# theadamsabra/last_torch

Hardware: AMD Instinct MI355X
Metric: lattice cells/s (B·T·U·|ctx|) at T=1000,U=100; 1/2/4/8-GPU scaling (higher is better)
Workload: dtype f32; 1 GPU; Log-semiring forward-backward (loss + dW), B=64/GPU, T=1000, U=100, V=32, FullNGram n=1 (C=33), fp32 (BASELINE configs[1]; configs[2] at 8 GPUs); batch_per_gpu=64, global_batch=64, frames=1000, labels=100, vocab=32, context_size=1, context_states=33, parallelism=utterance-sharded x1 (LPT), one RCCL all-reduce per step

## Files before the change

### last_torch_amd/csrc/lt_chunk.hip

```cpp
#include "lt_kernels.h"

#include <unistd.h>

#include <atomic>
#include <chrono>

namespace {

typedef float v16f __attribute__((ext_vector_type(16)));

constexpr float kEmin = 0x1p-88f;
constexpr int kRec = 1248;
constexpr int kRowT = 36;
constexpr int kChunkLds = 40 * 1024;
constexpr int kMargWaves = 4;
constexpr int kGrp = 7;
constexpr float kCert = 64.f;
constexpr int kAbWaves = 3;
constexpr unsigned kSpinMax = 1u << 20;
constexpr int kWalkPrio = 3;
constexpr int kDenPrio = 3;
constexpr int kASlot = 5 * 1024;
constexpr int kALdsBytes = 4 * 2 * kASlot;
constexpr int kWalkSlots = 3;
constexpr int kRecNi = (4 * kRec + 1023) / 1024;
constexpr int kWalkSlot = kRecNi * 1024;
constexpr int kWalkLds = 2 * kWalkSlots * kWalkSlot;
constexpr int kRecEj = 1152, kRecRt = 1184, kRecRho = 1216, kRecPi = 1217, kRecCs = 1218,
              kRecFlag = 1219, kRecN = 1220;

struct CkArgs {
  const unsigned char* W;
  const int* nfr;
  const int* labels;
  const int* nlab;
  const float* grad;
  float* rec;
  float* nb;
  int* uflag;
  float* abd;
  float* bbd;
  float* nabd;
  float* nbbd;
  float* cf;
  unsigned long long* ready;
  unsigned long long* prog;
  unsigned long long ep_tag, pg_tag;
  float* mid;
  float* loss;
  float* log_z;
  float* num;
  float* lz_out;
  float* num_out;
  void* dW;
  int B, T, U, V, C, R, FR, NP, NPG, PPL, CP;
  int L, K;
  int NGc;
  int nc, wpos;
  int nbs;
  int half;
  int cont;
  int local;
  int strict;
  int dbg;
  long long* stamps;
  long long FB;
  int a_slots, a_ni, a_slot_bytes, a_wave_bytes, a_off_rt, a_off_tab;
  int b_ni, b_slots, b_off_ra, b_off_rb, b_off_ga, b_off_gb, b_gslots, b_gslot, b_off_buf;
  int c_ni, c_off_ad, c_off_bd, c_off_an, c_off_bn, c_off_nw, c_off_fs, c_off_tab, c_off_cf,
      c_off_buf, c_off_fl, c_off_e, c_bytes;
};

LT_DEVINL float half_sum(float v) {
  auto p = __builtin_amdgcn_permlane32_swap(__float_as_int(v), __float_as_int(v), false, false);
  return __int_as_float(p[0]) + __int_as_float(p[1]);
}
LT_DEVINL float half_max(float v) {
  auto p = __builtin_amdgcn_permlane32_swap(__float_as_int(v), __float_as_int(v), false, false);
  float r;
  asm("v_max_f32 %0, %1, %2" : "=v"(r) : "v"(__int_as_float(p[0])), "v"(__int_as_float(p[1])));
  return r;
}
LT_DEVINL float from_prev(float v, float fill) {
  return __int_as_float(
      __builtin_amdgcn_update_dpp(__float_as_int(fill), __float_as_int(v), 0x138, 0xF, 0xF, false));
}
LT_DEVINL float rot_prev(float v) {
  return __int_as_float(__builtin_amdgcn_update_dpp(0, __float_as_int(v), 0x13C, 0xF, 0xF, false));
}
LT_DEVINL float rot_next(float v) {
  return __int_as_float(__builtin_amdgcn_update_dpp(0, __float_as_int(v), 0x134, 0xF, 0xF, false));
}

LT_DEVINL float safe_max(float m) { return __builtin_isfinite(m) ? m : 0.f; }
#ifdef LT_DIAG
#define CK_STAMP(k)                                                                  \
  do {                                                                               \
    if (a.stamps && !LT_ABL(a, 64 | 256) && threadIdx.x == 0)                         \
      a.stamps[(long long)blockIdx.x * 8 + (k)] = (long long)__builtin_amdgcn_s_memtime(); \
  } while (0)
#define CK_WSTAMP(k)                                                                 \
  do {                                                                               \
    if (a.stamps && LT_ABL(a, 64) && (threadIdx.x & 63) == 0)                         \
      a.stamps[(long long)b * 8 + (k)] = (long long)__builtin_amdgcn_s_memtime();     \
  } while (0)
#define CK_ASTAMP(k)                                                                 \
  do {                                                                               \
    if (a.stamps && LT_ABL(a, 256) && (threadIdx.x & 63) == 0)                        \
      a.stamps[(long long)a.B * a.K * 8 + (long long)id * 4 + (k)] =                  \
          (long long)__builtin_amdgcn_s_memtime();                                   \
  } while (0)
#else
#define CK_ASTAMP(k) \
  do {               \
  } while (0)
#define CK_WSTAMP(k) \
  do {               \
  } while (0)
#define CK_STAMP(k) \
  do {              \
  } while (0)
#endif
LT_DEVINL float max3_raw(float x, float y, float z) {
  float r;
  asm("v_max3_f32 %0, %1, %2, %3" : "=v"(r) : "v"(x), "v"(y), "v"(z));
  return r;
}
LT_DEVINL float first_lane(float v) {
  return __int_as_float(__builtin_amdgcn_readfirstlane(__float_as_int(v)));
}

LT_DEVINL int kstep(int s, int h) { return (s & 3) + 8 * (s >> 2) + 4 * h; }

template <bool BF16>
LT_DEVINL float ldsw(const unsigned char* fr, int e) {
  if constexpr (BF16) return __uint_as_float(((unsigned)((const unsigned short*)fr)[e]) << 16);
  else return ((const float*)fr)[e];
}

LT_DEVINL void dma_issue(const unsigned char* base, long long off, long long bytes,
                         unsigned lds_addr, int ni, int lane, int wave0 = 0, int nwaves = 1,
                         bool sc1 = false) {
  const long long a0 = off & ~15LL;
  const int n16 = (int)((off + bytes - a0 + 15) >> 4);
  for (int i = wave0; i < ni; i += nwaves) {
    int g = lane + 64 * i;
    g = g < n16 ? g : n16 - 1;
    if (sc1) glds16_sc1(base + a0 + 16LL * g, lds_addr + 1024u * i);
    else glds16(base + a0 + 16LL * g, lds_addr + 1024u * i);
  }
}

template <bool MAX>
LT_DEVINL float wred(float v) {
  if constexpr (MAX) v = dpp_max<3>(dpp_max<2>(dpp_max<1>(dpp_max<0>(v))));
  else v = dpp_add<3>(dpp_add<2>(dpp_add<1>(dpp_add<0>(v))));
  return __int_as_float(__builtin_amdgcn_readlane(__float_as_int(rows_fold<MAX>(v)), 63));
}
LT_DEVINL float wmax_u(float v) { return wred<true>(v); }
LT_DEVINL float wsum_u(float v) { return wred<false>(v); }

template <bool BF16>
LT_DEVINL float ldg(const unsigned char* base, long long e) {
  if constexpr (BF16) return __uint_as_float(((unsigned)((const unsigned short*)base)[e]) << 16);
  else return ((const float*)base)[e];
}

LT_DEVINL void string_offsets(const CkArgs& a, const int* lab, int u, int* boff, int* loff) {
  auto valid = [&](int y) { return y >= 1 && y <= a.V; };
  int ctx = 0, pc = 0;
  int j = min(u, a.U) - 1;
  for (; j >= 0; --j)
    if (valid(lab[j])) { ctx = lab[j]; break; }
  if (u >= 1) {
    if (j == u - 1) {
      for (int i = u - 2; i >= 0; --i)
        if (valid(lab[i])) { pc = lab[i]; break; }
    } else {
      pc = ctx;
    }
  }
  *boff = u < a.NP ? ctx * a.R : -1;
  if (u == 0 || u >= a.NP) {
    *loff = -1;
  } else {
    const int y = lab[u - 1];
    *loff = pc * a.R + (valid(y) ? y : 1);
  }
}

LT_DEVINL float lse2_b2(float x, float y) {
  const float m = fmaxf(x, y), n = fminf(x, y);
// ... 202 lines not shown
    const float dgv = (FULL || i < V) ? (noexp ? F.wdg : lt_exp_off(F.wdg, cl)) : 0.f;
    if (lane < 32) sdg[lane] = dgv;
    float A[16];
    float e0;
    if (noexp) {
#pragma unroll
      for (int s = 0; s < 16; ++s) A[s] = F.w[s];
      e0 = F.wr0;
    } else {
    const float ebl = lt_exp_off(F.wbl, cl);
    bool lnan = (lane <= V) && !(ebl >= 0.f);
    bool lwide = (lane <= V) && !(ebl >= kEmin);
#pragma unroll
    for (int s = 0; s < 16; ++s) {
      const bool live = FULL || (kstep(s, h) < V && i < V);
      const float e = lt_exp_off(F.w[s], cl);
      lnan = lnan || (live && !(e >= 0.f));
      lwide = lwide || (live && !(e >= kEmin));
      A[s] = live ? e : 0.f;
    }
    const float e0r = lt_exp_off(F.wr0, cl);
    e0 = (FULL || i < V) ? e0r : 0.f;
    lnan = lnan || ((FULL || i < V) && !(e0r >= 0.f));
    lwide = lwide || ((FULL || i < V) && !(e0r >= kEmin));
    if (!cfin || __builtin_amdgcn_ballot_w64(lnan)) bad = 2;
    else if (bad == 0 && __builtin_amdgcn_ballot_w64(lwide)) bad = 3;
    }
    const float w00 = F.w00;
    if (reload && !LT_ABL(a, 8192)) {
      wait_vmcnt(f + 2 < nt ? a.a_ni : 0);
      lds_frame<BF16, PPL, FULL>(aframe(f + 1), fo, F);
    }

    {
      float part = h ? 0.f : dgv * rt[i];
#pragma unroll
      for (int g = 0; g < 4; ++g) {
        const float4 r4 = *(const float4*)(rt + 8 * g + 4 * h);
        part = __builtin_fmaf(A[4 * g + 0], r4.x, part);
        part = __builtin_fmaf(A[4 * g + 1], r4.y, part);
        part = __builtin_fmaf(A[4 * g + 2], r4.z, part);
        part = __builtin_fmaf(A[4 * g + 3], r4.w, part);
      }
      const float y = half_sum(part);
      const float lam = pi;
      const int B0 = __builtin_isfinite(lam) ? max(rho, (int)floorf(lam)) : rho;
      float nr = ldexpf(y, max(rho - B0, -200)) + e0 * __builtin_amdgcn_exp2f(lam - (float)B0);
      nr = (FULL || i < V) ? nr : 0.f;
      int e;
      frexpf(wmax_u(lane < 32 ? nr : 0.f), &e);
      nr = ldexpf(nr, -e);
      rho = B0 + e;
      if (lane < 32) rt[lane] = nr;
    }
    pi += __builtin_fmaf(w00, kLog2e, -cl);
    csum += cl;

    if (LT_ABL(a, 2048)) return;
    v16f D = {};
#pragma unroll
    for (int s = 0; s < 16; ++s) D = __builtin_amdgcn_mfma_f32_32x32x2f32(A[s], X[s], D, 0, 0, 0);
#pragma unroll
    for (int g = 0; g < 4; ++g) {
      const float4 d4 = *(const float4*)(sdg + 8 * g + 4 * h);
      D[4 * g + 0] = __builtin_fmaf(d4.x, X[4 * g + 0], D[4 * g + 0]);
      D[4 * g + 1] = __builtin_fmaf(d4.y, X[4 * g + 1], D[4 * g + 1]);
      D[4 * g + 2] = __builtin_fmaf(d4.z, X[4 * g + 2], D[4 * g + 2]);
      D[4 * g + 3] = __builtin_fmaf(d4.w, X[4 * g + 3], D[4 * g + 3]);
    }
    float cm = fmaxf(max3_raw(D[0], D[1], D[2]), max3_raw(D[3], D[4], D[5]));
#pragma unroll
    for (int r = 6; r < 16; r += 2) cm = max3_raw(cm, D[r], D[r + 1]);
    cm = half_max(cm);
    int e;
    frexpf(cm, &e);
    e = cm > 0.f ? e : 0;
#pragma unroll
    for (int r = 0; r < 16; ++r) X[r] = ldexpf(D[r], -e);
    ej += e;
  };
  aissue(0);
  if (nt > 1) aissue(1);
  wait_vmcnt(nt > 1 ? a.a_ni : 0);
  lds_frame<BF16, PPL, FULL>(aframe(0), fo, fr);
  for (int f = 0; f < nt; ++f) step(fr, f, f + 1 < nt);
  if (lane < nt) a.cf[(long long)b * a.T + t0 + lane] = cfl_lane;
  CK_ASTAMP(2);

  const __amdgpu_buffer_rsrc_t rr = wt_rsrc(a.rec + (long long)id * kRec, 4 * kRec);
#pragma unroll
  for (int r = 0; r < 16; ++r) {
    st_wt(rr, kstep(r, h) * kRowT + i, X[r]);
  }
  if (lane < 32) {
    st_wt(rr, kRecEj + lane, ej);
    st_wt(rr, kRecRt + lane, rt[lane]);
  }
  bad = __builtin_amdgcn_readfirstlane(bad);
  if (lane == 0) {
    st_wt(rr, kRecRho, rho);
    st_wt(rr, kRecPi, pi);
    st_wt(rr, kRecCs, csum);
    st_wt(rr, kRecFlag, bad);
    st_wt(rr, kRecN, nt);
  }
  asm volatile("s_waitcnt vmcnt(0)" ::: "memory");
  CK_ASTAMP(3);
  const bool withhold = LT_ABL(a, 512) && b == 0 && k == 1;
  if (lane == 0 && !withhold)
    __hip_atomic_store((gu64*)(a.ready + id), a.ep_tag | (bad ? (unsigned)bad : 1u),
                       __ATOMIC_RELAXED, __HIP_MEMORY_SCOPE_AGENT);
}

LT_DEVINL unsigned long long poll_flag(const unsigned long long* p) {
  unsigned long long v;
  asm volatile("global_load_dwordx2 %0, %1, off sc1\n\ts_waitcnt vmcnt(0)" : "=v"(v) : "v"(p) : "memory");
  return v;
}
LT_DEVINL unsigned flag_state(unsigned long long v, unsigned long long tag) {
  return (v & ~3ull) == tag ? (unsigned)(v & 3) : 0u;
}
LT_DEVINL int prog_count(unsigned long long v, unsigned long long tag) {
  return (v & ~0xFFFFFFull) == tag ? (int)(v & 0xFFFFFF) : 0;
}
LT_DEVINL float4 ld_sc1x4(__amdgpu_buffer_rsrc_t r, int byte_off) {
  const v4u v = __builtin_amdgcn_raw_buffer_load_b128(r, byte_off, 0, 0x10);
  return make_float4(__uint_as_float(v.x), __uint_as_float(v.y), __uint_as_float(v.z),
                     __uint_as_float(v.w));
}
LT_DEVINL float ld_sc1(const float* p) {
  return __hip_atomic_load(p, __ATOMIC_RELAXED, __HIP_MEMORY_SCOPE_AGENT);
}
struct ChunkReady {
  const unsigned long long* f;
  unsigned long long tag;
  int lo, hi, Kl, ok, bad, strict;
  LT_DEVINL ChunkReady(const unsigned long long* flags, unsigned long long tg, int kl, int st)
      : f(flags), tag(tg), lo(kl), hi(-1), Kl(kl), ok(1), bad(0), strict(st) {}
  LT_DEVINL void take(unsigned v, int lane, int* c) {
    const unsigned long long m = __builtin_amdgcn_ballot_w64(v != 0);
    *c = m == ~0ull ? 64 : __builtin_ctzll(~m);
    const unsigned long long live = *c == 64 ? ~0ull : ((1ull << *c) - 1);
    if (__builtin_amdgcn_ballot_w64(v == 2u || (strict && v == 3u)) & live) bad = 1;
  }
  LT_DEVINL void timeout() {
    ok = 0;
    hi = Kl - 1;
    lo = 0;
  }
  LT_DEVINL void ensure_fwd(int k, int lane) {
    k = min(k, Kl - 1);
    for (unsigned spins = 0; k > hi; ++spins) {
      const int x = hi + 1 + lane;
      const unsigned v = flag_state(poll_flag(f + min(x, Kl - 1)), tag) & (x < Kl ? ~0u : 0u);
      int c;
      take(v, lane, &c);
      if (c) {
        hi += c;
      } else if (spins > kSpinMax) {
        timeout();
      } else {
        __builtin_amdgcn_s_sleep(4);
      }
    }
  }
  LT_DEVINL void ensure_bwd(int k, int lane) {
    k = max(k, 0);
    for (unsigned spins = 0; k < lo; ++spins) {
      const int x = lo - 1 - lane;
      const unsigned v = flag_state(poll_flag(f + max(x, 0)), tag) & (x >= 0 ? ~0u : 0u);
      int c;
      take(v, lane, &c);
      if (c) {
        lo -= c;
      } else if (spins > kSpinMax) {
        timeout();
      } else {
        __builtin_amdgcn_s_sleep(4);
      }
    }
  }
};

struct RecAlpha {
  float4 x[8];
  float rt, sc;
  float pi, cs;
};
LT_DEVINL void load_rec_alpha(const float* rc, int lane, int V, RecAlpha& r) {
#pragma unroll
  for (int g = 0; g < 8; ++g) r.x[g] = *(const float4*)(rc + (lane & 31) * kRowT + 4 * g);
  r.rt = rc[kRecRt + (lane & 31)];
  const int si = lane == 0 ? kRecRho : kRecEj + min(lane, 32) - 1;
  const int sc = ((const int*)rc)[si];
  r.sc = lane <= V ? (float)sc : 0.f;
  r.pi = rc[kRecPi];
  r.cs = rc[kRecCs];
}
struct RecBeta {
  float x[16];
// ... 123 lines not shown
      n[r][0] = g[r][0].x; n[r][1] = g[r][0].y; n[r][2] = g[r][0].z; n[r][3] = g[r][0].w;
      n[r][4] = g[r][1].x; n[r][5] = g[r][1].y; n[r][6] = g[r][1].z; n[r][7] = g[r][1].w;
    }
    if constexpr (FWD) {
#pragma unroll
      for (int r = 0; r < PPL; ++r)
#pragma unroll
        for (int d = 0; d < NB; ++d) tab[(lane + 64 * r + d) * TS + d] = v[r] + n[r][d];
    } else {
#pragma unroll
      for (int r = 0; r < PPL; ++r) sv[lane + 64 * r] = v[r];
    }
    __builtin_amdgcn_s_waitcnt(0xc07f);
    __builtin_amdgcn_wave_barrier();
    float x[PPL][NB];
#pragma unroll
    for (int r = 0; r < PPL; ++r)
#pragma unroll
      for (int d = 0; d < NB; ++d)
        x[r][d] = FWD ? tab[(lane + 64 * r) * TS + d] : n[r][d] + sv[lane + 64 * r + d];
    bload(qn, g);
    float vm = -kInf;
#pragma unroll
    for (int r = 0; r < PPL; ++r) {
      float m = x[r][0];
#pragma unroll
      for (int d = 1; d < NB; ++d) m = fmaxf(m, x[r][d]);
      const float ms = m == -kInf ? 0.f : m;
      float sum = 0.f;
#pragma unroll
      for (int d = 0; d < NB; ++d) sum += __builtin_amdgcn_exp2f(x[r][d] - ms);
      v[r] = lane + 64 * r < NPG ? ms + __builtin_amdgcn_logf(sum) : -kInf;
      vm = fmaxf(vm, v[r]);
    }
    {
      const float mv = wmax_u(vm);
      const float fl = __builtin_isfinite(mv) ? floorf(mv) : 0.f;
#pragma unroll
      for (int r = 0; r < PPL; ++r) v[r] -= fl;
      off += fl;
    }
    if (!FWD && q % NGc == 0) {
#pragma unroll
      for (int r = 0; r < PPL; ++r)
        if (lane + 64 * r < NPG) bd_store(dst + (long long)(q / NGc) * NPG + lane + 64 * r, v[r], wt);
      publish(Kh - q / NGc, false);
    }
    __builtin_amdgcn_wave_barrier();
  };
  const int cnt = q1 - q0;
  auto qof = [&](int n) { return FWD ? q0 + n : q1 - 1 - n; };
#pragma unroll
  for (int d = 0; d < D; ++d) bload(qof(d), gq[d]);
  const int nmain = cnt - cnt % D;
  for (int n0 = 0; n0 < nmain; n0 += D) {
#pragma unroll
    for (int d = 0; d < D; ++d) step(gq[d], qof(n0 + d), qof(n0 + d + D));
  }
#pragma unroll
  for (int d = 0; d < D; ++d)
    if (nmain + d < cnt) step(gq[d], qof(nmain + d), qof(nmain + d));
  if (ph == kWalkFirst) {
    if (FWD) {
#pragma unroll
      for (int r = 0; r < PPL; ++r)
        if (lane + 64 * r < NPG) dst[(long long)Kh * NPG + lane + 64 * r] = v[r];
      if (lane == 0) a.mid[2LL * b + 1] = off;
    }
    return;
  }
  publish(FWD ? (Kl - 1) - Kh : Kh, true);
  if constexpr (FWD) {
    float nv = -kInf;
#pragma unroll
    for (int r = 0; r < PPL; ++r)
      if (lane + 64 * r == nl) nv = v[r];
    nv = wmax_u(nv);
    if (lane == 0)
      *s_num = (nl >= 0 && nl <= a.U) ? (float)(((double)off + (double)nv) * 0.6931471805599453)
                                       : -kInf;
  }
}

template <int PPL, int D>
LT_DEVINL void combine_role(const CkArgs& a, int b, int wave, unsigned char* dyn, int ph) {
  const WalkLds wl = walk_lds(dyn);
  const int lane = threadIdx.x & 63;
  int nf = a.nfr[b];
  nf = nf < 0 ? 0 : (nf > a.T ? a.T : nf);
  const int Kl = (nf + a.L - 1) / a.L;
  const int Kh = Kl / 2;
  const int V = a.V, C = a.C, CP = a.CP;
  const int nl = a.nlab[b];
  if (ph == kWalkRest && a.uflag[b]) return;
  if (threadIdx.x == 0) *wl.bad = 0;
  __syncthreads();
  CK_WSTAMP(2 * wave);
  ChunkReady rd(a.ready + (long long)b * a.K, a.ep_tag, Kl, a.strict);
  if (ph == kWalkRest) {
    rd.lo = 0;
    rd.hi = Kl - 1;
  }
  const bool wt = ph == kWalkRest;

  const unsigned ring_a = lds_base_addr(wl.ring) + (unsigned)(wave * kWalkSlots * kWalkSlot);
  const unsigned char* ring = wl.ring + wave * kWalkSlots * kWalkSlot;
  auto issue_rec = [&](int k, int n) {
    const int kc = min(max(k, 0), Kl - 1);
    dma_issue((const unsigned char*)a.rec, ((long long)b * a.K + kc) * (kRec * 4), kRec * 4,
              ring_a + (unsigned)((n % kWalkSlots) * kWalkSlot), kRecNi, lane, 0, 1, true);
  };
  auto wait_rec = [&](int n) {
    wait_vmcnt(n < kWalkSlots ? kRecNi * (kWalkSlots - 1) + n : (kRecNi + 1) * kWalkSlots - kRecNi);
  };
  auto slot = [&](int n) { return (const float*)(ring + (n % kWalkSlots) * kWalkSlot); };

  if (wave == 0 && !a.local && !LT_ABL(a, 1)) {
    float* bc = wl.bc;
    float* dst = a.abd + (long long)b * (a.K + 1) * CP;
    const int k0 = ph == kWalkRest ? Kh : 0, k1 = ph == kWalkFirst ? Kh : Kl;
    float al, O;
    if (ph == kWalkRest) {
      const float x = dst[(long long)Kh * CP + min(lane, C - 1)];
      al = lane < C ? x : -kInf;
      O = a.mid[2LL * b];
    } else {
      al = lane == 0 ? 0.f : -kInf;
      O = 0.f;
      if (lane < C) dst[lane] = al;
    }
    int pub = 0;
    if (k1 > k0) {
      rd.ensure_fwd(k0 + kWalkSlots - 1, lane);
      for (int n = 0; n < kWalkSlots; ++n) issue_rec(k0 + n, n);
    }
    for (int k = k0; k < k1; ++k) {
      const int n = k - k0;
      wait_rec(n);
      RecAlpha R;
      load_rec_alpha(slot(n), lane, V, R);
      const float x = lane < C ? al + R.sc : -kInf;
      const float M = safe_max(wmax_u(x));
      const float av = lane < C ? __builtin_amdgcn_exp2f(x - M) : 0.f;
      if (lane >= 1 && lane <= 32) bc[lane - 1] = av;
      if (lane == 0) bc[32] = av;
      __builtin_amdgcn_s_waitcnt(0xc07f);
      __builtin_amdgcn_wave_barrier();
      float s0 = 0.f, s1 = 0.f;
#pragma unroll
      for (int g = 0; g < 8; g += 2) {
        const float4 a0 = *(const float4*)(bc + 4 * g);
        const float4 a1 = *(const float4*)(bc + 4 * g + 4);
        s0 = __builtin_fmaf(R.x[g].x, a0.x, s0);
        s1 = __builtin_fmaf(R.x[g + 1].x, a1.x, s1);
        s0 = __builtin_fmaf(R.x[g].y, a0.y, s0);
        s1 = __builtin_fmaf(R.x[g + 1].y, a1.y, s1);
        s0 = __builtin_fmaf(R.x[g].z, a0.z, s0);
        s1 = __builtin_fmaf(R.x[g + 1].z, a1.z, s1);
        s0 = __builtin_fmaf(R.x[g].w, a0.w, s0);
        s1 = __builtin_fmaf(R.x[g + 1].w, a1.w, s1);
      }
      s0 = __builtin_fmaf(R.rt, bc[32], s0);
      const float cs = R.cs, pi = R.pi;
      __builtin_amdgcn_s_waitcnt(0xc07f);
      rd.ensure_fwd(k + kWalkSlots, lane);
      issue_rec(k + kWalkSlots, n + kWalkSlots);
      const float fl = floorf(M);
      const float nq = (M - fl) + __builtin_amdgcn_logf(s0 + s1);
      const float n0 = first_lane(al) + pi - fl;
      O += cs + fl;
      const float sh = from_prev(nq, -kInf);
      al = lane == 0 ? n0 : (lane < C ? sh : -kInf);
      if (lane < C) bd_store(dst + (long long)(k + 1) * CP + lane, al, wt);
      if (wt && k + 1 - Kh - pub >= kProgStep && k + 1 < k1) {
        prog_publish(a, b, 0, k + 1 - Kh, lane);
        pub = k + 1 - Kh;
// ... 53 lines not shown
      rd.ensure_bwd(k - kWalkSlots, lane);
      issue_rec(k - kWalkSlots, n + kWalkSlots);
      const float fl = floorf(Mc);
      const float tot = half_sum(p0 + p1);
      const float nj = (Mc - fl) + ej + __builtin_amdgcn_logf(tot);
      const float rsum = wsum_u(rp);
      const float rterm = (Mc - fl) + rho + __builtin_amdgcn_logf(rsum);
      const float nb0 = lse2_b2(first_lane(be) + pi - fl, rterm);
      const float sh = from_prev(nj, -kInf);
      be = lane == 0 ? nb0 : (lane < C ? sh : -kInf);
      if (lane < C) bd_store(dst + (long long)k * CP + lane, be, wt);
      if (wt && Kh - k - pub >= kProgStep && k > k0) {
        prog_publish(a, b, 1, Kh - k, lane);
        pub = Kh - k;
      }
      __builtin_amdgcn_wave_barrier();
    }
    if (wt) prog_publish(a, b, 1, Kh - k0, lane);
  } else if (wave == 2 && !LT_ABL(a, 2) && !LT_ABL(a, 128)) {
    num_walk<PPL, true, D>(a, b, lane, nf, Kl, nl, wl.nva, wl.num, rd, ph);
  } else if (wave == 3 && !LT_ABL(a, 2)) {
    num_walk<PPL, false, D>(a, b, lane, nf, Kl, nl, wl.nvb, nullptr, rd, ph);
  }
  if (lane == 0 && (rd.bad || !rd.ok)) *wl.bad = 1;
  CK_WSTAMP(2 * wave + 1);
  __syncthreads();
  if (ph == kWalkFirst) {
    if (threadIdx.x == 0) a.uflag[b] = *wl.bad ? 1 : 0;
    return;
  }
  if (*wl.bad) {
    if (threadIdx.x == 0) a.uflag[b] = 1;
    return;
  }
  if (threadIdx.x == 0) {
    const float lz = a.local ? 0.f : *wl.lz;
    const float nm = *wl.num;
    if (ph == kWalkRest && ((!a.local && !__builtin_isfinite(lz)) || !__builtin_isfinite(nm)))
      a.uflag[b] = 1;
    else if (ph == kWalkFull)
      a.uflag[b] = 0;
    a.log_z[b] = lz;
    a.num[b] = nm;
    if (a.lz_out) a.lz_out[b] = lz;
    if (a.num_out) a.num_out[b] = nm;
    a.loss[b] = a.local ? -nm : lz - nm;
  }
}

template <int PPL>
constexpr int kWalkD = PPL == 1 ? 8 : (kAbWaves > 3 ? 4 : 5);
template <int PPL>
constexpr int kWalkDc = PPL == 1 ? 4 : 3;

template <bool BF16, int PPL, bool FULL>
__global__ __launch_bounds__(256, kAbWaves) void ck_ab_kernel(const CkArgs a) {
  const int nc = a.nc;
  const int wave = __builtin_amdgcn_readfirstlane(threadIdx.x >> 6);
  int x = blockIdx.x;
  if (x >= a.wpos && x < a.wpos + nc) {
    extern __shared__ __attribute__((aligned(16))) unsigned char ck_dyn[];
    __builtin_amdgcn_s_setprio(kWalkPrio);
    combine_role<PPL, kWalkD<PPL>>(a, x - a.wpos, wave, ck_dyn, a.half ? kWalkFirst : kWalkFull);
    return;
  }
  if (x >= a.wpos) x -= nc;
  const long long j = (long long)x * 4 + wave;
  const int m = (int)(j / (2 * a.B));
  const int r = (int)(j - (long long)m * 2 * a.B);
  const int b = r < a.B ? r : r - a.B;
  int nf = a.nfr[b];
  nf = nf < 0 ? 0 : (nf > a.T ? a.T : nf);
  const int Kl = (nf + a.L - 1) / a.L;
  const int k = r < a.B ? m : Kl - 1 - m;
  if (r < a.B ? m > Kl - 1 - m : Kl - 1 - m <= m) return;
  transfer_role<BF16, PPL, FULL>(a, b, k, wave);
}

template <int PPL>
__global__ __launch_bounds__(256) void ck_combine_kernel(const CkArgs a) {
  extern __shared__ __attribute__((aligned(16))) unsigned char ck_dyn[];
  combine_role<PPL, kWalkD<PPL>>(a, blockIdx.x, __builtin_amdgcn_readfirstlane(threadIdx.x >> 6),
                                 ck_dyn, a.half ? kWalkFirst : kWalkFull);
}

LT_DEVINL void gather_tables(const CkArgs& a, int b, int* lab, int* boff, int* loff, int tid,
                             int nthr) {
  for (int j = tid; j < a.U; j += nthr) lab[j] = a.labels[(long long)b * a.U + j];
  __syncthreads();
  for (int u = tid; u < a.NPG; u += nthr) {
    int bo, lo;
    string_offsets(a, lab, u, &bo, &lo);
    boff[u] = bo < 0 ? 0 : bo;
    loff[u] = lo;
  }
}

template <bool BF16>
LT_DEVINL void store_dw(void* dW, long long e, float v) {
  if constexpr (BF16) ((unsigned short*)dW)[e] = f2bf(v);
  else ((float*)dW)[e] = v;
}

constexpr int kFs = 8, kFsMa = 0, kFsA0 = 1, kFsMb = 2, kFsB0 = 3, kFsW00 = 4;
constexpr int kFlA = 1, kFlB = 2, kFlNA = 4, kFlNB = 8, kFlAll = 15, kFlNT = 16;

template <bool BF16, int PPL, bool FULL, int LC = 0>
__global__ __launch_bounds__(64 * kMargWaves, kMargWaves / 2) void ck_marg_kernel(const CkArgs a) {
  static_assert(LC == 0 || FULL, "a compile-time chunk length needs V = 32");
  extern __shared__ __attribute__((aligned(16))) unsigned char lds[];
  const int tid = threadIdx.x, lane = tid & 63;
  const int wave = __builtin_amdgcn_readfirstlane(tid >> 6);
  constexpr int kFbC = 33 * 33 * (BF16 ? 2 : 4);
  constexpr int kNiC = ((LC * kFbC + 30) / 16 + 63) / 64;
  constexpr int kAdC = kNiC * 1024, kBdC = kAdC + ((4 * LC * 36 + 15) & ~15);
  const int cL = LC ? LC : a.L;
  const long long cFB = LC ? (long long)kFbC : a.FB;
  const int cNi = LC ? kNiC : a.c_ni;
  const int cOffAd = LC ? kAdC : a.c_off_ad, cOffBd = LC ? kBdC : a.c_off_bd;
  if (a.cont && (int)blockIdx.x < a.B) {
    CK_STAMP(0);
    __builtin_amdgcn_s_setprio(kWalkPrio);
    combine_role<PPL, kWalkDc<PPL>>(a, blockIdx.x, wave, lds, kWalkRest);
    CK_STAMP(4);
    return;
  }
  const int c = a.cont ? (int)blockIdx.x - a.B : (int)blockIdx.x;
  const int j = c / a.B, b = c - j * a.B;
  if (a.uflag[b]) return;
  int nf = a.nfr[b];
  nf = nf < 0 ? 0 : (nf > a.T ? a.T : nf);
  const int Kl = (nf + cL - 1) / cL, Kh = Kl / 2;
  const int k = j < 2 * Kh ? ((j & 1) ? Kh - 1 - (j >> 1) : Kh + (j >> 1)) : j;
  const int t0 = k * cL;
  const int tend = min(t0 + cL, a.T);
  const int t1 = max(t0, min(t0 + cL, nf));
  const int V = FULL ? 32 : a.V, C = V + 1, R = V + 1, FR = C * R, CP = FULL ? 36 : a.CP;
  const int NPG = a.NPG, NP = a.NP;
  const int FRP = (FR + 3) & ~3;
  float g = a.grad ? a.grad[b] : 1.f;
  if (!a.cont) {
    const float lz = a.log_z[b], nm = a.num[b];
    if ((!a.local && !__builtin_isfinite(lz)) || __builtin_isnan(nm)) {
      if (tid == 0) a.uflag[b] = 1;
      return;
    }
    if (!__builtin_isfinite(nm)) g = 0.f;
  }
  const long long e0 = ((long long)b * a.T + t0) * FR;
  if (t1 <= t0 || g == 0.f) {
    const long long n = (long long)(tend - t0) * FR;
    for (long long e = tid; e < n; e += blockDim.x) store_dw<BF16>(a.dW, e0 + e, 0.f);
    return;
  }
  const int nt = t1 - t0;
  CK_STAMP(0);
  const int role = (wave + (int)(blockIdx.x >> 3)) & 3;
  const int hs = (nt + 1) / 2;
  const long long off = e0 * (BF16 ? 2 : 4);
  dma_issue(a.W, off, (long long)nt * cFB, lds_base_addr(lds), cNi, lane, wave, kMargWaves);
  unsigned char* wch = lds + (off & 15);
  float* xa = (float*)(lds + cOffAd);
  float* xb = (float*)(lds + cOffBd);
  float* an = (float*)(lds + a.c_off_an);
  float* bn = (float*)(lds + a.c_off_bn);
  float2* nw = (float2*)(lds + a.c_off_nw);
  float* fs = (float*)(lds + a.c_off_fs);
  int* boff = (int*)(lds + a.c_off_tab);
  int* loff = boff + NPG;
  int* labs = loff + NPG;
  float* buf = (float*)(lds + a.c_off_buf) + 64 * wave;
  float* cfl = (float*)(lds + a.c_off_cf);
  int* fl = (int*)(lds + a.c_off_fl);
  int* ford = fl + cL;
  int* njob = ford + cL;
  int* cert_fail = njob + 1;
  auto init_flags = [&](int t) {
    if (t < nt) {
      fl[t] = 0;
      const int mid = (nt - 1) / 2;
      const int k = (t + 1) / 2;
      ford[t] = (t & 1) ? mid + k : mid - k;
    }
    if (t == 0) {
      *njob = 0;
      *cert_fail = 0;
    }
  };
  if (tid < nt) cfl[tid] = a.cf[(long long)b * a.T + t0 + tid];
  if (a.cont && tid == 0) {
    const int need_a = k - Kh, need_b = Kh - (k + 1);
    const unsigned long long* pg = a.prog + 4LL * b;
    int ok = 1;
    for (unsigned spins = 0;; ++spins) {
      bool done = true;
      if (need_a > 0)
        done = (a.local || prog_count(poll_flag(pg + 0), a.pg_tag) >= need_a) &&
               prog_count(poll_flag(pg + 2), a.pg_tag) >= need_a;
      if (done && need_b > 0)
        done = (a.local || prog_count(poll_flag(pg + 1), a.pg_tag) >= need_b) &&
               prog_count(poll_flag(pg + 3), a.pg_tag) >= need_b;
      if (done) break;
      if (spins > kSpinMax) {
        ok = 0;
        break;
      }
      __builtin_amdgcn_s_sleep(2);
    }
    CK_STAMP(6);
    fl[2 * cL + 2] = ok;
  }
  gather_tables(a, b, labs, boff, loff, tid, blockDim.x);
  wait_vmcnt(0);
  __syncthreads();
  if (a.cont && !fl[2 * cL + 2]) {
    if (tid == 0) a.uflag[b] = 1;
    return;
  }
  CK_STAMP(1);
  auto wrow = [&](int f) -> const unsigned char* { return wch + f * cFB; };
  auto eptr = [&](int f) -> float* {
    return BF16 ? (float*)(lds + a.c_off_e) + f * FRP : (float*)(wch + f * cFB);
  };
  auto ew = [](float w, float cl) -> float {
    return __builtin_amdgcn_exp2f(__builtin_fmaf(w, kLog2e, -cl));
  };
  {
    constexpr int PW = 64 * PPL, FPP = 64 * kMargWaves / PW, NU = PPL == 1 ? 2 : 3;
    const int u = tid & (PW - 1), f0 = tid / PW;
    const int uc = min(u, NPG - 1);
    const int ob = boff[uc], ol = max(loff[uc], 0);
    const bool inb = u < NP, inl = u >= 1 && u < NP;
    const int FBi = (int)cFB;
    float2 g2[NU];
#pragma unroll
    for (int i = 0; i < NU; ++i) {
      const unsigned char* fr = wch + min(FPP * i + f0, nt - 1) * FBi;
      const float wb = ldsw<BF16>(fr, ob), wl = ldsw<BF16>(fr, ol);
      g2[i] = make_float2(inb ? wb * kLog2e : -kInf, inl ? wl * kLog2e : -kInf);
    }
    for (int f = FPP * NU + f0; f < nt; f += FPP) {
      const unsigned char* fr = wch + f * FBi;
      const float wb = ldsw<BF16>(fr, ob), wl = ldsw<BF16>(fr, ol);
      if (u < NPG) nw[f * NPG + u] = make_float2(inb ? wb * kLog2e : -kInf, inl ? wl * kLog2e : -kInf);
    }
#pragma unroll
    for (int i = 0; i < NU; ++i) {
      const int f = FPP * i + f0;
      if (f < nt && u < NPG) nw[f * NPG + u] = g2[i];
    }
  }
  if (tid < nt) fs[tid * kFs + kFsW00] = ldsw<BF16>(wch + tid * cFB, 0) * kLog2e;
  init_flags(tid);
  __syncthreads();
  CK_STAMP(5);

  auto mark = [&](int f, int bit) {
    __builtin_amdgcn_fence(__ATOMIC_RELEASE, "workgroup");
    if (lane == 0) __hip_atomic_fetch_or(fl + f, bit, __ATOMIC_RELAXED, __HIP_MEMORY_SCOPE_WORKGROUP);
  };
  auto mark_all = [&](int bit) {
    for (int f = 0; f < nt; ++f) mark(f, bit);
  };
  auto wait_bits = [&](int f, int want) {
    for (;;) {
      const int bits = __builtin_amdgcn_readfirstlane(
          __hip_atomic_load(fl + f, __ATOMIC_RELAXED, __HIP_MEMORY_SCOPE_WORKGROUP));
      if ((bits & want) == want) break;
      __builtin_amdgcn_s_sleep(1);
    }
    __builtin_amdgcn_fence(__ATOMIC_ACQUIRE, "workgroup");
  };

  if (role < 2) __builtin_amdgcn_s_setprio(kDenPrio);
  if (role == 0 && !a.local && !LT_ABL(a, 4)) {
    const int q = lane & 31, h = lane >> 5;
    const int qe = min(q, V - 1) + 1;
    const bool core = lane >= 1 && lane <= V;
    const float* xp = a.abd + ((long long)b * (a.K + 1) + k) * CP + min(lane, C - 1);
    const float xr = ld_sc1(xp);
    const float x0 = lane < C ? xr : -kInf;
    float a0 = first_lane(x0);
    float S = wmax_u(core ? x0 : -kInf);
    float al = (core && S != -kInf) ? __builtin_amdgcn_exp2f(x0 - S) : 0.f;
    auto get_e = [&](int f, float* e, float& e32, float& eb, float& w00) {
      const unsigned char* fr = wrow(f);
      float* ef = eptr(f);
      const float cl = cfl[f];
      w00 = fs[f * kFs + kFsW00];
      if (f < hs) {
#pragma unroll
        for (int m = 0; m < 16; ++m) e[m] = ldsw<BF16>(fr, min(16 * h + m, C - 1) * R + qe);
        e32 = ldsw<BF16>(fr, min(32, C - 1) * R + qe);
        eb = ldsw<BF16>(fr, qe * R);
#pragma unroll
// ... 303 lines not shown
        const bool live = yl && (m < 16 ? 16 * h + m < C : (h == 1 && C > 32));
        const float v = t[m] * ra[m] * xby;
        t[m] = live ? v : 0.f;
        sum += t[m];
      }
      sum = wsum_u(sum);
      const float* fsf = fs + f * kFs;
      const float base = fsf[kFsMa] + fsf[kFsMb] + cfl[f];
      const float v00 = fsf[kFsA0] + fsf[kFsW00] + fsf[kFsB0];
      const float zl = lse2_b2(base + __builtin_amdgcn_logf(sum), v00);
      if (!(base - zl <= kCert) && lane == 0) *cert_fail = 1;
      const float mult = g * __builtin_amdgcn_exp2f(base - zl);
      const float m00 = g * __builtin_amdgcn_exp2f(v00 - zl);
      __builtin_amdgcn_s_waitcnt(0xc07f);
      __builtin_amdgcn_wave_barrier();
#pragma unroll
      for (int m = 0; m < NROW; ++m) {
        const int p = m < 16 ? 16 * h + m : 32;
        if (y + 1 < R && (m < 16 ? p < C : (h == 1 && C > 32))) fb[p * R + y + 1] = t[m] * mult;
      }
      if (colc) fb[pc * R] = lane == 0 ? m00 : tc * mult;
    } else {
      __builtin_amdgcn_s_waitcnt(0xc07f);
      __builtin_amdgcn_wave_barrier();
      for (int e = lane; e < FR; e += 64) fb[e] = 0.f;
    }
#pragma unroll
    for (int r = 0; r < PPL; ++r) {
      const int u = lane + 64 * r;
      if (u < NP) {
        atomicAdd(fb + bo[r], sb[r]);
        if (u >= 1) atomicAdd(fb + lo[r], sl[r]);
      }
    }
    __builtin_amdgcn_s_waitcnt(0xc07f);
    __builtin_amdgcn_wave_barrier();
    if constexpr (BF16) {
      unsigned short* fo = (unsigned short*)(wch + f * cFB);
      for (int e = lane; e < FR; e += 64) fo[e] = f2bf(fb[e]);
    }
  }
  __syncthreads();
  if (*cert_fail) {
    if (tid == 0) a.uflag[b] = 1;
    return;
  }
  CK_STAMP(3);
  {
    const long long es = BF16 ? 2 : 4;
    const long long bytes = (long long)nt * cFB;
    unsigned char* gdst = (unsigned char*)a.dW + off;
    const long long head = min((long long)((16 - (off & 15)) & 15), bytes);
    const long long body = (bytes - head) & ~15LL;
    const unsigned char* src = wch;
    for (long long x = tid; x < head / es; x += blockDim.x) {
      if constexpr (BF16) ((unsigned short*)gdst)[x] = ((const unsigned short*)src)[x];
      else ((float*)gdst)[x] = ((const float*)src)[x];
    }
    const uint4* s16 = (const uint4*)(src + head);
    uint4* d16 = (uint4*)(gdst + head);
    for (long long x = tid; x < body / 16; x += blockDim.x) d16[x] = s16[x];
    for (long long x = head + body + tid * es; x < bytes; x += blockDim.x * es) {
      if constexpr (BF16) *(unsigned short*)(gdst + x) = *(const unsigned short*)(src + x);
      else *(float*)(gdst + x) = *(const float*)(src + x);
    }
  }
  CK_STAMP(4);
  {
    const long long n = (long long)(tend - t1) * FR;
    const long long base = e0 + (long long)nt * FR;
    for (long long e = tid; e < n; e += blockDim.x) store_dw<BF16>(a.dW, base + e, 0.f);
  }
}

}

namespace {

int ck_env(const char* name, int dflt) { return lt_impl::tune_int(name, dflt); }
long long up256(long long x) { return (x + 255) & ~255LL; }
int al16(long long x) { return (int)((x + 15) & ~15LL); }

struct CkLayout {
  size_t uflag, lz, num, abd, bbd, nabd, nbbd, cf, mid, state;
  size_t ready, rec, nb, f_alpha, f_an, f_loss, f_lz, f_num, f_side, scratch;
};

int ck_plan(const lt_problem* pb, int local_norm, CkArgs* a, CkLayout* w) {
  memset(a, 0, sizeof(*a));
  const int V = pb->vocab_size;
  const bool bf16 = pb->weight_dtype == LT_DTYPE_BF16;
  const int es = bf16 ? 2 : 4;
  a->B = pb->batch; a->T = pb->max_frames; a->U = pb->max_labels;
  a->V = V; a->C = V + 1; a->R = V + 1; a->FR = a->C * a->R;
  a->NP = a->U + 1; a->NPG = (a->NP + 1) & ~1; a->PPL = (a->NPG + 63) / 64;
  a->CP = (a->C + 3) & ~3;
  a->local = local_norm ? 1 : 0;
#ifdef LT_DIAG
  a->dbg = ck_env("LT_CK_DBG", 0);
  if (const char* sp = lt_impl::tune_str("LT_CK_STAMPS")) a->stamps = (long long*)strtoull(sp, nullptr, 0);
#endif
  a->FB = (long long)a->FR * es;
  const long long n16f = (a->FB + 30) / 16;
  a->a_ni = (int)((n16f + 63) / 64);
  a->a_slots = 3;
  a->a_slot_bytes = a->a_ni * 1024;
  a->a_off_rt = a->a_slots * a->a_slot_bytes;
  a->a_off_tab = a->a_off_rt + 128;
  a->a_wave_bytes = al16(a->a_off_tab + 8LL * a->NPG);
  a->b_ni = (kRec * 4 + 15 + 1023) / 1024;
  a->b_slots = 4;
  a->b_off_ra = 0;
  a->b_off_rb = a->b_slots * a->b_ni * 1024;
  a->b_gslot = 1024;
  a->b_gslots = 16;
  a->b_off_ga = a->b_off_rb + a->b_slots * a->b_ni * 1024;
  a->b_off_gb = a->b_off_ga + a->b_gslots * a->b_gslot;
  a->b_off_buf = a->b_off_gb + a->b_gslots * a->b_gslot;
  auto c_bytes = [&](int L, CkArgs* t) {
    const long long n16 = ((long long)L * a->FB + 30) / 16;
    t->c_ni = (int)((n16 + 63) / 64);
    int off = t->c_ni * 1024;
    t->c_off_ad = off; off += al16(4LL * L * a->CP);
    t->c_off_bd = off; off += al16(4LL * L * a->CP);
    t->c_off_an = off; off += al16(4LL * L * a->NPG);
    t->c_off_bn = off; off += al16(4LL * L * a->NPG);
    t->c_off_nw = off; off += al16(8LL * L * a->NPG);
    t->c_off_fs = off; off += al16(4LL * L * kFs);
    t->c_off_tab = off; off += al16(8LL * a->NPG + 4LL * a->U);
    t->c_off_cf = off; off += al16(4LL * L);
    t->c_off_buf = off; off += 4 * 64 * 4;
    t->c_off_fl = off; off += al16(4LL * (2 * L + 3));
    t->c_off_e = off; off += bf16 ? al16(4LL * L * ((a->FR + 3) & ~3)) : 0;
    return off;
  };
  int L = std::max(1, std::min(32, ck_env("LT_CHUNK_LEN", 32)));
  const int budget = ck_env("LT_CHUNK_LDS", kChunkLds);
  while (L > 4 && c_bytes(L, a) > budget) --L;
  if (c_bytes(L, a) > 160 * 1024) return lt_impl::set_error(LT_EUNSUPPORTED, "chunk: LDS");
  a->c_bytes = c_bytes(L, a);
  a->L = L;
  a->K = std::max(1, (a->T + L - 1) / L);
  if (a->K >= (1 << 24)) return lt_impl::set_error(LT_EUNSUPPORTED, "chunk: too many frames");
  a->NGc = (L + kGrp - 1) / kGrp;
  const long long B = a->B, K = a->K, T = a->T;
  size_t o = 0;
  w->uflag = o; o += up256(4 * B);
  w->lz = o; o += up256(4 * B);
  w->num = o; o += up256(4 * B);
  w->abd = o; o += up256(4 * B * (K + 1) * a->CP);
  w->bbd = o; o += up256(4 * B * (K + 1) * a->CP);
  w->nabd = o; o += up256(4 * B * (K + 1) * a->NPG);
  w->nbbd = o; o += up256(4 * B * (K + 1) * a->NPG);
  w->cf = o; o += up256(4 * B * T);
  w->mid = o; o += up256(8 * B);
  w->state = o;
  size_t s = 0;
  w->ready = s; s += up256(8LL * B * K + 32LL * B);
  w->rec = s; s += up256(4LL * B * K * kRec);
  a->nbs = (a->NGc * (kGrp + 1) * a->NPG + 31) & ~31;
  w->nb = s; s += up256(4LL * B * K * a->nbs);
  const size_t fwd = s;
  s = 0;
  w->f_alpha = s; s += up256(4LL * B * T * a->C);
  w->f_an = s; s += up256(4LL * B * T * a->NP);
  w->f_loss = s; s += up256(4 * B);
  w->f_lz = s; s += up256(4 * B);
  w->f_num = s; s += up256(4 * B);
  w->f_side = s; s += up256((long long)lt_impl::serial_side_bytes(pb, local_norm));
  w->scratch = std::max(fwd, s);
  return LT_OK;
}

void ck_bind(CkArgs* a, const CkLayout& w, void* state, void* scratch) {
  char* st = (char*)state;
  char* sc = (char*)scratch;
  a->uflag = (int*)(st + w.uflag);
  a->log_z = (float*)(st + w.lz);
  a->num = (float*)(st + w.num);
  a->abd = (float*)(st + w.abd);
  a->bbd = (float*)(st + w.bbd);
  a->nabd = (float*)(st + w.nabd);
  a->nbbd = (float*)(st + w.nbbd);
  a->cf = (float*)(st + w.cf);
  a->mid = (float*)(st + w.mid);
  a->rec = sc ? (float*)(sc + w.rec) : nullptr;
  a->nb = sc ? (float*)(sc + w.nb) : nullptr;
  a->ready = sc ? (unsigned long long*)(sc + w.ready) : nullptr;
  a->prog = sc ? (unsigned long long*)(sc + w.ready) + (long long)a->B * a->K : nullptr;
}

int ck_launch(const void* k, int grid, int lds, hipStream_t st, const CkArgs& a,
              int threads = 256) {
  if (grid <= 0) return LT_OK;
  hipError_t e = hipFuncSetAttribute(k, hipFuncAttributeMaxDynamicSharedMemorySize, lds);
  if (e != hipSuccess) return lt_impl::set_error(LT_EHIP, hipGetErrorString(e));
  void* args[] = {(void*)&a};
  e = hipLaunchKernel(k, dim3(grid), dim3(threads), args, lds, st);
  if (e == hipSuccess) e = hipGetLastError();
  if (e != hipSuccess) return lt_impl::set_error(LT_EHIP, hipGetErrorString(e));
  return LT_OK;
}

int ck_check(const lt_problem* pb) {
  if (!pb) return lt_impl::set_error(LT_EINVAL, "null problem");
  if (pb->batch < 0 || pb->max_frames < 0 || pb->max_labels < 0)
    return lt_impl::set_error(LT_EINVAL, "negative dimension");
  if (pb->weight_dtype != LT_DTYPE_F32 && pb->weight_dtype != LT_DTYPE_BF16)
    return lt_impl::set_error(LT_EINVAL, "weight_dtype must be LT_DTYPE_F32 or LT_DTYPE_BF16");
  if (!lt_impl::chunk_eligible(pb))
    return lt_impl::set_error(LT_EUNSUPPORTED,
                              "chunked path: FullNGram n = 1, vocab_size <= 32, labels < 128");
  return LT_OK;
}

const void* ck_kernel_ab(int ppl, bool bf16, bool full) {
  if (full)
    return ppl == 1 ? (bf16 ? (const void*)ck_ab_kernel<true, 1, true>
                            : (const void*)ck_ab_kernel<false, 1, true>)
                    : (bf16 ? (const void*)ck_ab_kernel<true, 2, true>
                            : (const void*)ck_ab_kernel<false, 2, true>);
  return ppl == 1 ? (bf16 ? (const void*)ck_ab_kernel<true, 1, false>
                          : (const void*)ck_ab_kernel<false, 1, false>)
                  : (bf16 ? (const void*)ck_ab_kernel<true, 2, false>
                          : (const void*)ck_ab_kernel<false, 2, false>);
}
const void* ck_kernel_b(int ppl) {
  return ppl == 1 ? (const void*)ck_combine_kernel<1> : (const void*)ck_combine_kernel<2>;
}
int ck_cus() {
  static int cus[64];
  int dev = 0;
  if (hipGetDevice(&dev) != hipSuccess || dev < 0 || dev >= 64) return 0;
  if (!cus[dev] && hipDeviceGetAttribute(&cus[dev], hipDeviceAttributeMultiprocessorCount, dev) !=
                       hipSuccess)
    cus[dev] = 0;
  return cus[dev];
}
unsigned long long ck_seed() {
  unsigned long long z = (unsigned long long)std::chrono::steady_clock::now().time_since_epoch().count();
  z ^= (unsigned long long)getpid() << 32;
  z ^= (unsigned long long)(uintptr_t)&ck_cus;
  return z;
}
void ck_tags(CkArgs& a) {
  static std::atomic<unsigned long long> ctr{ck_seed()};
  unsigned long long z = ctr.fetch_add(0x9E3779B97F4A7C15ull) + 0x9E3779B97F4A7C15ull;
  z = (z ^ (z >> 30)) * 0xBF58476D1CE4E5B9ull;
  z = (z ^ (z >> 27)) * 0x94D049BB133111EBull;
  z ^= z >> 31;
  a.ep_tag = ((z >> 2) | (1ull << 61)) << 2;
  a.pg_tag = ((z & 0xFFFFFFFFFFull) | (1ull << 39)) << 24;
}
int ck_launch_ab(CkArgs& a, bool bf16, hipStream_t st) {
  ck_tags(a);
  if (lt_impl::stream_capturing(st)) {
    const hipError_t e =
        hipMemsetAsync(a.ready, 0, 8ull * a.B * a.K + 32ull * a.B, st);
    if (e != hipSuccess) return lt_impl::set_error(LT_EHIP, hipGetErrorString(e));
  }
  const bool fuse = a.B <= ck_cus() && ck_env("LT_CHUNK_FUSE", 1) != 0;
  a.nc = fuse ? a.B : 0;
  const long long items = 2LL * a.B * ((a.K + 1) / 2);
  const long long nwa = (items + 3) / 4;
  const int at = ck_env("LT_CHUNK_WALK_AT", std::max(0, 100 - 4800 / std::max(a.B, 1)));
  a.wpos = (int)(nwa * std::min(std::max(at, 0), 100) / 100);
  int rc = ck_launch(ck_kernel_ab(a.PPL, bf16, a.V == 32), (int)(a.nc + nwa),
                     std::max(fuse ? kWalkLdsBytes : 0, kALdsBytes), st, a);
// ... 185 lines not shown
```

Measured before the change: 690.5 billion cells/s.

## Precompute label offset tables in combine pass and prefetch them with progress flags

Moves the per-utterance string-offset table computation out of the marginal kernel into the combine role, which writes it to a global state buffer. The marginal kernel then DMA-loads the precomputed table into LDS. Wave 0 issues the progress-flag and cf loads early alongside the weight DMA, and only falls back to the spin-poll loop when a ballot shows a flag is not yet satisfied. This is meant to take the label gather, the extra __syncthreads and the serial polling off the marginal kernel's startup path, at the cost of extra global state and shifting the table work into the combine kernel.

```diff
diff --git a/last_torch_amd/csrc/lt_chunk.hip b/last_torch_amd/csrc/lt_chunk.hip
--- a/last_torch_amd/csrc/lt_chunk.hip
+++ b/last_torch_amd/csrc/lt_chunk.hip
@@ -43,6 +43,7 @@
   float* nabd;
   float* nbbd;
   float* cf;
+  int* tab;
   unsigned long long* ready;
   unsigned long long* prog;
   unsigned long long ep_tag, pg_tag;
@@ -107,7 +108,7 @@
 #define CK_ASTAMP(k)                                                                 \
   do {                                                                               \
     if (a.stamps && LT_ABL(a, 256) && (threadIdx.x & 63) == 0)                        \
-      a.stamps[(long long)a.B * a.K * 8 + (long long)id * 4 + (k)] =                  \
+      a.stamps[(long long)a.B * a.K * 8 + (long long)id * 8 + (k)] =                  \
           (long long)__builtin_amdgcn_s_memtime();                                   \
   } while (0)
 #else
@@ -476,6 +477,7 @@
   aissue(0);
   if (nt > 1) aissue(1);
   wait_vmcnt(nt > 1 ? a.a_ni : 0);
+  CK_ASTAMP(4);
   lds_frame<BF16, PPL, FULL>(aframe(0), fo, fr);
   for (int f = 0; f < nt; ++f) step(fr, f, f + 1 < nt);
   if (lane < nt) a.cf[(long long)b * a.T + t0 + lane] = cfl_lane;
@@ -510,6 +512,20 @@
   unsigned long long v;
   asm volatile("global_load_dwordx2 %0, %1, off sc1\n\ts_waitcnt vmcnt(0)" : "=v"(v) : "v"(p) : "memory");
   return v;
+}
+LT_DEVINL unsigned long long early_flag(const unsigned long long* p) {
+  unsigned long long v;
+  asm volatile("global_load_dwordx2 %0, %1, off sc1" : "=v"(v) : "v"(p) : "memory");
+  return v;
+}
+LT_DEVINL float early_f32(const float* p) {
+  float v;
+  asm volatile("global_load_dword %0, %1, off" : "=v"(v) : "v"(p) : "memory");
+  return v;
+}
+template <class T>
+LT_DEVINL void landed(T& v) {
+  asm volatile("" : "+v"(v) : : "memory");
 }
 LT_DEVINL unsigned flag_state(unsigned long long v, unsigned long long tag) {
   return (v & ~3ull) == tag ? (unsigned)(v & 3) : 0u;
@@ -799,6 +815,18 @@
   }
 }
 
+LT_DEVINL void gather_tables(const CkArgs& a, int b, int tid, int nthr) {
+  const int* lab = a.labels + (long long)b * a.U;
+  int* boff = a.tab + (long long)b * 2 * a.NPG;
+  int* loff = boff + a.NPG;
+  for (int u = tid; u < a.NPG; u += nthr) {
+    int bo, lo;
+    string_offsets(a, lab, u, &bo, &lo);
+    boff[u] = bo < 0 ? 0 : bo;
+    loff[u] = lo;
+  }
+}
+
 template <int PPL, int D>
 LT_DEVINL void combine_role(const CkArgs& a, int b, int wave, unsigned char* dyn, int ph) {
   const WalkLds wl = walk_lds(dyn);
@@ -809,6 +837,7 @@
   const int Kh = Kl / 2;
   const int V = a.V, C = a.C, CP = a.CP;
   const int nl = a.nlab[b];
+  if (ph != kWalkRest) gather_tables(a, b, threadIdx.x, blockDim.x);
   if (ph == kWalkRest && a.uflag[b]) return;
   if (threadIdx.x == 0) *wl.bad = 0;
   __syncthreads();
@@ -1028,18 +1057,6 @@
   extern __shared__ __attribute__((aligned(16))) unsigned char ck_dyn[];
   combine_role<PPL, kWalkD<PPL>>(a, blockIdx.x, __builtin_amdgcn_readfirstlane(threadIdx.x >> 6),
                                  ck_dyn, a.half ? kWalkFirst : kWalkFull);
-}
-
-LT_DEVINL void gather_tables(const CkArgs& a, int b, int* lab, int* boff, int* loff, int tid,
-                             int nthr) {
-  for (int j = tid; j < a.U; j += nthr) lab[j] = a.labels[(long long)b * a.U + j];
-  __syncthreads();
-  for (int u = tid; u < a.NPG; u += nthr) {
-    int bo, lo;
-    string_offsets(a, lab, u, &bo, &lo);
-    boff[u] = bo < 0 ? 0 : bo;
-    loff[u] = lo;
-  }
 }
 
 template <bool BF16>
@@ -1104,7 +1121,6 @@
   const int role = (wave + (int)(blockIdx.x >> 3)) & 3;
   const int hs = (nt + 1) / 2;
   const long long off = e0 * (BF16 ? 2 : 4);
-  dma_issue(a.W, off, (long long)nt * cFB, lds_base_addr(lds), cNi, lane, wave, kMargWaves);
   unsigned char* wch = lds + (off & 15);
   float* xa = (float*)(lds + cOffAd);
   float* xb = (float*)(lds + cOffBd);
@@ -1114,7 +1130,6 @@
   float* fs = (float*)(lds + a.c_off_fs);
   int* boff = (int*)(lds + a.c_off_tab);
   int* loff = boff + NPG;
-  int* labs = loff + NPG;
   float* buf = (float*)(lds + a.c_off_buf) + 64 * wave;
   float* cfl = (float*)(lds + a.c_off_cf);
   int* fl = (int*)(lds + a.c_off_fl);
@@ -1133,30 +1148,46 @@
       *cert_fail = 0;
     }
   };
-  if (tid < nt) cfl[tid] = a.cf[(long long)b * a.T + t0 + tid];
-  if (a.cont && tid == 0) {
+  if (wave == 0) {
     const int need_a = k - Kh, need_b = Kh - (k + 1);
     const unsigned long long* pg = a.prog + 4LL * b;
-    int ok = 1;
-    for (unsigned spins = 0;; ++spins) {
-      bool done = true;
-      if (need_a > 0)
-        done = (a.local || prog_count(poll_flag(pg + 0), a.pg_tag) >= need_a) &&
-               prog_count(poll_flag(pg + 2), a.pg_tag) >= need_a;
-      if (done && need_b > 0)
-        done = (a.local || prog_count(poll_flag(pg + 1), a.pg_tag) >= need_b) &&
-               prog_count(poll_flag(pg + 3), a.pg_tag) >= need_b;
-      if (done) break;
-      if (spins > kSpinMax) {
-        ok = 0;
-        break;
-      }
-      __builtin_amdgcn_s_sleep(2);
+    unsigned long long pv = 0;
+    if (a.cont) pv = early_flag(pg + (lane & 3));
+    float cfv = early_f32(a.cf + (long long)b * a.T + t0 + min(lane, nt - 1));
+    dma_issue((const unsigned char*)a.tab, 8LL * b * NPG, 8LL * NPG,
+              lds_base_addr(lds + a.c_off_tab), 1, lane);
+    dma_issue(a.W, off, (long long)nt * cFB, lds_base_addr(lds), cNi, lane, 0, kMargWaves);
+    wait_vmcnt((cNi + kMargWaves - 1) / kMargWaves);
+    landed(pv);
+    landed(cfv);
+    if (lane < nt) cfl[lane] = cfv;
+    if (a.cont) {
+      const int w = lane & 3, need = (w & 1) ? need_b : need_a;
+      const bool have = need <= 0 || (a.local && w < 2) || prog_count(pv, a.pg_tag) >= need;
+      int ok = 1;
+      if (__builtin_amdgcn_ballot_w64(!have) && tid == 0) {
+        for (unsigned spins = 0;; ++spins) {
+          bool done = true;
+          if (need_a > 0)
+            done = (a.local || prog_count(poll_flag(pg + 0), a.pg_tag) >= need_a) &&
+                   prog_count(poll_flag(pg + 2), a.pg_tag) >= need_a;
+          if (done && need_b > 0)
+            done = (a.local || prog_count(poll_flag(pg + 1), a.pg_tag) >= need_b) &&
+                   prog_count(poll_flag(pg + 3), a.pg_tag) >= need_b;
+          if (done) break;
+          if (spins > kSpinMax) {
+            ok = 0;
+            break;
+          }
+          __builtin_amdgcn_s_sleep(2);
+        }
+      }
+      if (tid == 0) fl[2 * cL + 2] = ok;
     }
     CK_STAMP(6);
-    fl[2 * cL + 2] = ok;
-  }
-  gather_tables(a, b, labs, boff, loff, tid, blockDim.x);
+  } else {
+    dma_issue(a.W, off, (long long)nt * cFB, lds_base_addr(lds), cNi, lane, wave, kMargWaves);
+  }
   wait_vmcnt(0);
   __syncthreads();
   if (a.cont && !fl[2 * cL + 2]) {
@@ -1626,7 +1657,7 @@
 int al16(long long x) { return (int)((x + 15) & ~15LL); }
 
 struct CkLayout {
-  size_t uflag, lz, num, abd, bbd, nabd, nbbd, cf, mid, state;
+  size_t uflag, lz, num, abd, bbd, nabd, nbbd, cf, mid, tab, state;
   size_t ready, rec, nb, f_alpha, f_an, f_loss, f_lz, f_num, f_side, scratch;
 };
 
@@ -1698,6 +1729,7 @@
   w->nbbd = o; o += up256(4 * B * (K + 1) * a->NPG);
   w->cf = o; o += up256(4 * B * T);
   w->mid = o; o += up256(8 * B);
+  w->tab = o; o += up256(8 * B * a->NPG);
   w->state = o;
   size_t s = 0;
   w->ready = s; s += up256(8LL * B * K + 32LL * B);
@@ -1728,6 +1760,7 @@
   a->nbbd = (float*)(st + w.nbbd);
   a->cf = (float*)(st + w.cf);
   a->mid = (float*)(st + w.mid);
+  a->tab = (int*)(st + w.tab);
   a->rec = sc ? (float*)(sc + w.rec) : nullptr;
   a->nb = sc ? (float*)(sc + w.nb) : nullptr;
   a->ready = sc ? (unsigned long long*)(sc + w.ready) : nullptr;
```

Result: faster. 718.2 billion cells/s, median of 6 (+4.0%).
